# kopacja/rho2sdf.jl

Hardware: AMD Instinct MI355X
Metric: Mvoxels/s SDF extract on 512^3 grid over 100k HEX8; max|err| vs ref (higher is better)
Workload: dtype f64

## Files before the change

### include/rho2sdf_hip.h

```cpp
#ifndef RHO2SDF_HIP_H
#define RHO2SDF_HIP_H

#include <stddef.h>
#include <stdint.h>

#ifdef __cplusplus
extern "C" {
#endif

#define R2S_VERSION 100

#define R2S_OK 0
#define R2S_ERR_ARG (-1)
#define R2S_ERR_NO_DEVICE (-2)
#define R2S_ERR_HIP (-3)
#define R2S_ERR_UNSUPPORTED (-4)
#define R2S_ERR_NOMEM (-5)

#define R2S_HEX8 0
#define R2S_TET4 1

typedef struct {
    double aabb_min[3];
    double aabb_max[3];
// ... 95 lines not shown
void r2s_host_free(void *p);

typedef struct r2s_plan r2s_plan;

int r2s_plan_create(int32_t device, r2s_plan **out);
void r2s_plan_destroy(r2s_plan *plan);

#define R2S_OUT_DIST 1
#define R2S_OUT_SIGN 2
#define R2S_OUT_SDF 4
#define R2S_OUT_XP 8

int r2s_plan_run_dev(r2s_plan *plan, const double *dX, int64_t nnp, const int64_t *dIEN, int64_t nel,
                     const double *d_rho_n, double rho_t, const r2s_grid *grid,
                     const r2s_params *params, int64_t k_begin, int64_t k_end, int32_t mode,
                     double *d_dist, double *d_sign, double *d_sdf, double *d_xp, void *stream,
                     r2s_stats *stats);

int r2s_plan_pack_tiles_dev(r2s_plan *plan, const double *d_local_sdf, double *d_payload, uint32_t *d_ids,
                            int64_t capacity_tiles, int64_t *n_tiles_out, void *stream);
int r2s_unpack_tiles_dev(const double *d_payload, const uint32_t *d_ids, int64_t n_tiles, const r2s_grid *grid,
                         double *d_volume, void *stream);
int r2s_fill_dev(double *d, int64_t n, double value, void *stream);
int r2s_plan_pack_tiles2_dev(r2s_plan *plan, const double *d_local_sdf, double *d_payload, uint32_t *d_ids,
                             int64_t capacity_full, uint64_t *d_masks, uint32_t *d_mask_ids, int64_t capacity_mask,
                             int64_t *n_full_out, int64_t *n_mask_out, void *stream);
int r2s_unpack_masks_dev(const uint64_t *d_masks, const uint32_t *d_mask_ids, int64_t n_tiles, const r2s_grid *grid,
                         double magnitude, double *d_volume, void *stream);

int r2s_unpack_segments_dev(const double *d_buf, int32_t world, int64_t seglen, int64_t cap_full, int64_t cap_mask,
                            const r2s_grid *grid, double magnitude, double *d_volume, void *stream);


int r2s_mesh_volume(const double *X, int64_t nnp, const int64_t *IEN, int64_t nel, int32_t elem_type,
                    const double *rho_e, int32_t device, double *V_domain, double *V_frac);

int r2s_dense_in_nodes(const double *X, int64_t nnp, const int64_t *IEN, int64_t nel, int32_t elem_type,
                       const double *rho_e, int32_t device, double *rho_n_out);

int r2s_find_threshold(const double *X, int64_t nnp, const int64_t *IEN, int64_t nel, const double *rho_n,
                       double target_volume, double tol, int32_t maxit, int32_t device, double *rho_t_out,
                       int32_t *iters_out);

int r2s_find_threshold_et(const double *X, int64_t nnp, const int64_t *IEN, int64_t nel, int32_t elem_type,
                          const double *rho_n, double target_volume, double tol, int32_t maxit, int32_t device,
                          double *rho_t_out, int32_t *iters_out);
// ... 124 lines not shown
```

### rho2sdf.jl_amd/_lib.py

```python
import ctypes
import os

_HERE = os.path.dirname(os.path.abspath(__file__))
LIB_PATH = os.environ.get("R2S_LIB_OVERRIDE") or os.path.join(_HERE, "librho2sdf_hip.so")

c_double_p = ctypes.POINTER(ctypes.c_double)
c_int64_p = ctypes.POINTER(ctypes.c_int64)
c_float_p = ctypes.POINTER(ctypes.c_float)
c_int32_p = ctypes.POINTER(ctypes.c_int32)
OPT_EXTRACT_SURFACE = 0


class R2SGrid(ctypes.Structure):
    _fields_ = [("aabb_min", ctypes.c_double * 3), ("aabb_max", ctypes.c_double * 3),
                ("N", ctypes.c_int64 * 3), ("cell_size", ctypes.c_double), ("ngp", ctypes.c_int64)]


class R2SParams(ctypes.Structure):
    _fields_ = [("band_factor", ctypes.c_double), ("elem_type", ctypes.c_int32),
                ("device", ctypes.c_int32), ("zstride", ctypes.c_int32), ("zphase", ctypes.c_int32),
                ("n_gpus", ctypes.c_int32), ("true_min", ctypes.c_int32), ("sign_no_inner", ctypes.c_int32),
                ("reserved_", ctypes.c_int32)]


# ... 45 lines not shown
_P = ctypes.c_void_p
_MESH = [c_double_p, ctypes.c_int64, c_int64_p, ctypes.c_int64]
_COMMON = _MESH + [c_double_p, ctypes.c_double, ctypes.POINTER(R2SGrid), ctypes.POINTER(R2SParams)]
SYMBOLS = [
    ("r2s_version", ctypes.c_int, []),
    ("r2s_last_error", ctypes.c_char_p, []),
    ("r2s_device_count", ctypes.c_int, []),
    ("r2s_default_params", None, [ctypes.POINTER(R2SParams)]),
    ("r2s_grid_make", ctypes.c_int, [c_double_p, c_double_p, ctypes.c_int64, ctypes.c_int64,
                                     ctypes.POINTER(R2SGrid)]),
    ("r2s_auto_grid", ctypes.c_int, _MESH + [ctypes.c_int32, ctypes.POINTER(R2SGrid), c_double_p]),
    ("r2s_eval_distances", ctypes.c_int, _COMMON + [c_double_p, c_double_p, ctypes.POINTER(R2SStats)]),
    ("r2s_sign_detection", ctypes.c_int, _COMMON + [c_double_p, ctypes.POINTER(R2SStats)]),
    ("r2s_sdf", ctypes.c_int, _COMMON + [c_double_p, ctypes.POINTER(R2SStats)]),
    ("r2s_plan_create", ctypes.c_int, [ctypes.c_int32, ctypes.POINTER(_P)]),
    ("r2s_plan_destroy", None, [_P]),
    ("r2s_plan_run_dev", ctypes.c_int,
     [_P, _P, ctypes.c_int64, _P, ctypes.c_int64, _P, ctypes.c_double, ctypes.POINTER(R2SGrid),
      ctypes.POINTER(R2SParams), ctypes.c_int64, ctypes.c_int64, ctypes.c_int32, _P, _P, _P, _P, _P,
      ctypes.POINTER(R2SStats)]),
    ("r2s_plan_pack_tiles_dev", ctypes.c_int, [_P, _P, _P, _P, ctypes.c_int64, c_int64_p, _P]),
    ("r2s_unpack_tiles_dev", ctypes.c_int, [_P, _P, ctypes.c_int64, ctypes.POINTER(R2SGrid), _P, _P]),
    ("r2s_fill_dev", ctypes.c_int, [_P, ctypes.c_int64, ctypes.c_double, _P]),
    ("r2s_plan_pack_tiles2_dev", ctypes.c_int, [_P, _P, _P, _P, ctypes.c_int64, _P, _P, ctypes.c_int64, c_int64_p,
                                                c_int64_p, _P]),
    ("r2s_unpack_masks_dev", ctypes.c_int, [_P, _P, ctypes.c_int64, ctypes.POINTER(R2SGrid), ctypes.c_double, _P, _P]),
    ("r2s_unpack_segments_dev", ctypes.c_int, [_P, ctypes.c_int32, ctypes.c_int64, ctypes.c_int64, ctypes.c_int64,
                                               ctypes.POINTER(R2SGrid), ctypes.c_double, _P, _P]),
    ("r2s_mesh_volume", ctypes.c_int, _MESH + [ctypes.c_int32, c_double_p, ctypes.c_int32, c_double_p, c_double_p]),
    ("r2s_dense_in_nodes", ctypes.c_int, _MESH + [ctypes.c_int32, c_double_p, ctypes.c_int32, c_double_p]),
    ("r2s_find_threshold", ctypes.c_int, _MESH + [c_double_p, ctypes.c_double, ctypes.c_double, ctypes.c_int32,
                                                  ctypes.c_int32, c_double_p, ctypes.POINTER(ctypes.c_int32)]),
    ("r2s_find_threshold_et", ctypes.c_int, _MESH + [ctypes.c_int32, c_double_p, ctypes.c_double, ctypes.c_double,
                                                     ctypes.c_int32, ctypes.c_int32, c_double_p,
                                                     ctypes.POINTER(ctypes.c_int32)]),
    ("r2s_isocontour_volume", ctypes.c_int, _MESH + [ctypes.c_int32, c_double_p, ctypes.c_double, ctypes.c_int32,
                                                     c_double_p]),
    ("r2s_default_options", None, [ctypes.POINTER(R2SOptions)]),
    ("r2s_rho2sdf", ctypes.c_int, _MESH + [c_double_p, ctypes.POINTER(R2SOptions), ctypes.POINTER(R2SGrid), c_double_p,
                                           c_double_p, c_double_p, c_float_p, ctypes.POINTER(R2SRunInfo)]),
    ("r2s_last_host_phases", None, [c_double_p]),
    ("r2s_host_alloc", ctypes.c_void_p, [ctypes.c_size_t]),
    ("r2s_host_free", None, [ctypes.c_void_p]),
    ("r2s_remove_artifacts", ctypes.c_int, [c_double_p, ctypes.POINTER(R2SGrid), ctypes.c_double, ctypes.c_double,
                                            ctypes.c_int32, c_int64_p]),
    ("r2s_remove_artifacts_dev", ctypes.c_int, [_P, ctypes.POINTER(R2SGrid), ctypes.c_double, ctypes.c_double, _P,
# ... 101 lines not shown
```

### rho2sdf.jl_amd/csrc/rho2sdf_hip.hip

```cpp
#include <hip/hip_runtime.h>

#include <algorithm>
#include <cmath>
#include <cstdarg>
#include <cstddef>
#include <cstdio>
#include <cstring>
#include <initializer_list>
#include <utility>
#include <string>
#include <vector>

#include "../../include/rho2sdf_hip.h"
#include "r2s_common.hpp"
#include "r2s_device_math.hpp"

#include <type_traits>

using namespace r2s;

__constant__ int c_hex_isn[6][4] = {{0, 3, 2, 1}, {0, 1, 5, 4}, {1, 2, 6, 5},
                                    {2, 3, 7, 6}, {3, 0, 4, 7}, {4, 5, 6, 7}};

#define SCAN_BLOCK 256
#define SCAN_ITEMS 16
#define SCAN_TILE (SCAN_BLOCK * SCAN_ITEMS)

struct ScanPair {
    const uint32_t* in[2];
    uint32_t* out[2];
    uint32_t* sums[2];
};
__global__ void __launch_bounds__(SCAN_BLOCK) scan_block_kernel(ScanPair sp, int64_t n)
{
    __shared__ uint32_t wave_sums[SCAN_BLOCK / 64];
    const uint32_t* __restrict__ in = sp.in[blockIdx.y];
    uint32_t* __restrict__ out = sp.out[blockIdx.y];
    uint32_t* __restrict__ block_sums = sp.sums[blockIdx.y];
    const int64_t base = (int64_t)blockIdx.x * SCAN_TILE + (int64_t)threadIdx.x * SCAN_ITEMS;
    uint32_t v[SCAN_ITEMS], sum = 0;
#pragma unroll
    for (int i = 0; i < SCAN_ITEMS; ++i) {
        v[i] = (base + i < n) ? in[base + i] : 0u;
        sum += v[i];
    }
    const int lane = threadIdx.x & 63, wave = threadIdx.x >> 6;
    uint32_t incl = sum;
#pragma unroll
    for (int off = 1; off < 64; off <<= 1) {
        uint32_t t = __shfl_up(incl, off, 64);
        if (lane >= off) incl += t;
    }
    if (lane == 63) wave_sums[wave] = incl;
    __syncthreads();
    uint32_t wave_off = 0, total = 0;
#pragma unroll
    for (int w = 0; w < SCAN_BLOCK / 64; ++w) {
        if (w < wave) wave_off += wave_sums[w];
        total += wave_sums[w];
    }
    uint32_t run = wave_off + incl - sum;
#pragma unroll
    for (int i = 0; i < SCAN_ITEMS; ++i) {
        if (base + i < n) out[base + i] = run;
        run += v[i];
    }
    if (threadIdx.x == 0 && block_sums) block_sums[blockIdx.x] = total;
}

__global__ void scan_add_kernel(ScanPair sp, int64_t n)
{
    uint32_t* __restrict__ out = sp.out[blockIdx.y];
    const int64_t i = (int64_t)blockIdx.x * SCAN_TILE + threadIdx.x;
    const uint32_t add = sp.sums[blockIdx.y][blockIdx.x];
#pragma unroll
    for (int k = 0; k < SCAN_ITEMS; ++k) {
        int64_t j = i + (int64_t)k * SCAN_BLOCK;
        if (j < n) out[j] += add;
    }
}

struct ZeroSet {
    uint32_t* p[4];
    int64_t nwords[4];
};
__global__ void zero_many_kernel(ZeroSet z)
{
    uint32_t* __restrict__ p = z.p[blockIdx.y];
    const int64_t n = z.nwords[blockIdx.y];
    for (int64_t i = (int64_t)blockIdx.x * blockDim.x + threadIdx.x; i < n; i += (int64_t)gridDim.x * blockDim.x) p[i] = 0u;
}
static void zero_many(hipStream_t st, std::initializer_list<std::pair<void*, size_t>> bufs)
{
    ZeroSet z;
    unsigned nb = 0;
    int64_t mx = 0;
    for (const auto& b : bufs) {
        z.p[nb] = static_cast<uint32_t*>(b.first);
        z.nwords[nb] = (int64_t)((b.second + 3) / 4);
        mx = std::max(mx, z.nwords[nb]);
        nb++;
    }
    for (unsigned i = nb; i < 4; ++i) { z.p[i] = nullptr; z.nwords[i] = 0; }
    const unsigned gx = (unsigned)std::min<int64_t>((mx + 1023) / 1024, 2048);
    if (nb && gx) zero_many_kernel<<<dim3(gx, nb), 256, 0, st>>>(z);
}

struct ReadBack {
    const uint32_t* src[8];
    uint32_t n[8];
    uint32_t dst[8];
    int cnt = 0;
    void add(const uint32_t* p, uint32_t words, uint32_t at) { src[cnt] = p; n[cnt] = words; dst[cnt] = at; ++cnt; }
};
struct SpecExpect {
    uint32_t v[16];
    uint32_t on;
};
__global__ void read_back_kernel(ReadBack rb, uint32_t* __restrict__ host, SpecExpect ex, uint32_t* __restrict__ abort_flag)
{
    const int q = threadIdx.x >> 3, w = threadIdx.x & 7;
    if (q < rb.cnt && (uint32_t)w < rb.n[q]) {
        const uint32_t v = rb.src[q][w];
        host[rb.dst[q] + w] = v;
        if (ex.on && v != ex.v[rb.dst[q] + w]) *abort_flag = 1u;
    }
// ... 1355 lines not shown
                    x[2] = grid_coord(g, 2, slab_global_k(sl, kl));
                    inv_map_hex8(E, x, xi);
                    const double m = fmax(fabs(xi[0]), fmax(fabs(xi[1]), fabs(xi[2])));
                    double val = INFINITY;
                    if (m < 1.01) {
                        hex8_shape(xi, N);
                        double rho = 0.0;
#pragma unroll
                        for (int k = 0; k < 8; ++k) rho += N[k] * E.r[k];
                        val = (rho >= rho_t) ? m : -m;
                    }
                    res[tile_slot(st_off, tb, i, j, kl)] = val;
                }
            }
        }
        c = seg_end;
        if (c < c_end) {
            do { ++lo; } while (chunk_off[lo + 1] <= c);
        }
    }
}

#define AT_ITEMS 8
__global__ void __launch_bounds__(256) active_tiles_kernel(const uint32_t* __restrict__ band_cnt,
                                                           const uint32_t* __restrict__ sign_cnt,
                                                           const uint8_t* __restrict__ hot, uint32_t ntiles,
                                                           uint32_t* __restrict__ active_band,
                                                           uint32_t* __restrict__ active_sign,
                                                           uint32_t* __restrict__ active_any,
                                                           uint32_t* __restrict__ active_sonly,
                                                           const uint8_t* __restrict__ tri,
                                                           uint32_t* __restrict__ active_lean,
                                                           uint32_t* __restrict__ active_tri,
                                                           uint32_t* __restrict__ counters)
{
    __shared__ uint32_t s_cnt[6][AT_ITEMS][4], s_base[6], s_max[2];
    if (threadIdx.x < 2) s_max[threadIdx.x] = 0;
    const int lane = threadIdx.x & 63, wave = threadIdx.x >> 6;
    const unsigned long long below = (1ull << lane) - 1ull;
    const uint32_t t0 = blockIdx.x * (256u * AT_ITEMS);
    uint32_t mxb = 0, mxs = 0;
    uint32_t flags[AT_ITEMS];
#pragma unroll
    for (int i = 0; i < AT_ITEMS; ++i) {
        const uint32_t t = t0 + (uint32_t)i * 256u + threadIdx.x;
        const bool in = t < ntiles;
        const uint32_t bc = in ? band_cnt[t] : 0u, sc = in ? sign_cnt[t] : 0u;
        const bool f[3] = {bc != 0, sc != 0 && hot[t] != 0, false};
        const bool ft = f[0] && tri[t] != 0;
        const bool fl[6] = {f[0], f[1], f[0] || f[1], f[1] && !f[0], f[0] && !ft, ft};
        uint32_t fb = 0;
#pragma unroll
        for (int l = 0; l < 6; ++l) {
            const unsigned long long m = __ballot(fl[l]);
            if (lane == 0) s_cnt[l][i][wave] = (uint32_t)__popcll(m);
            fb |= fl[l] ? (1u << l) : 0u;
        }
        flags[i] = fb;
        if (fl[0] && bc > mxb) mxb = bc;
        if (fl[1] && sc > mxs) mxs = sc;
    }
    __syncthreads();
    if (mxb > 64u) atomicMax(&s_max[0], mxb);
    if (mxs > 64u) atomicMax(&s_max[1], mxs);
    if (threadIdx.x < 6) {
        const int idx[6] = {1, 2, 5, 6, 10, 11};
        uint32_t n = 0;
        for (int i = 0; i < AT_ITEMS; ++i)
            for (int w = 0; w < 4; ++w) {
                const uint32_t c = s_cnt[threadIdx.x][i][w];
// ... 377 lines not shown
__global__ void __launch_bounds__(256) unpack_segments_masks_kernel(const double* __restrict__ buf, int64_t seglen, uint32_t cap_full,
                                                                   uint32_t cap_mask, int nx, int ny, int nz, double magnitude,
                                                                   double* __restrict__ volume)
{
    const double* __restrict__ seg = buf + (int64_t)blockIdx.y * seglen;
    const int64_t nf = reinterpret_cast<const int64_t*>(seg)[0], nm = reinterpret_cast<const int64_t*>(seg)[1];
    const uint32_t w = __builtin_amdgcn_readfirstlane((blockIdx.x * blockDim.x + threadIdx.x) >> 6);
    if (nf < 0 || nf > (int64_t)cap_full || nm < 0 || nm > (int64_t)cap_mask || (int64_t)w >= nm) return;
    const uint64_t* __restrict__ masks = reinterpret_cast<const uint64_t*>(seg + 2 + (int64_t)cap_full * 64 + (cap_full + 1) / 2);
    const uint32_t* __restrict__ ids = reinterpret_cast<const uint32_t*>(masks + cap_mask);
    const int lane = threadIdx.x & 63;
    const int ntx = (nx + 3) / 4, nty = (ny + 3) / 4;
    const uint32_t t = ids[w];
    const int tx = t % ntx, ty = (t / ntx) % nty, tz = t / (ntx * nty);
    const int i = tx * 4 + (lane & 3), j = ty * 4 + ((lane >> 2) & 3), k = tz * 4 + (lane >> 4);
    if (i < nx && j < ny && k < nz) volume[((int64_t)k * ny + j) * nx + i] = ((masks[w] >> lane) & 1ull) ? magnitude : -magnitude;
}

struct r2s_plan {
    int device = 0;
    int n_cu = 256;
    DevBuf deg, ine_ptr, ine, cursor, erec, cls, fmask, nitems, item_off, items;
    DevBuf band_cnt, band_off, band_raw, band_ent, sign_cnt, sign_off, sign_raw, sign_ent;
    DevBuf active, active_sign, active_any, active_sonly, active_lean, active_tri, tri, hot, counters, scan_tmp[3], scan_tmp2[3], nchunks, chunk_off, iso_res, iso_res_xp, strag;
    DevBuf perm, wchunks, hardflag;
    DevBuf sbox, s_nchunks, s_chunk_off, sres;
    DevBuf nstore, store_off, s_nstore, s_store_off;
    SlabInfo last_s;
    GridDev last_g;
    uint32_t last_n_any = 0, last_n_band = 0, last_n_sonly = 0;
    bool has_last = false;
    uint32_t* h_pinned = nullptr;
    uint32_t* d_pinned = nullptr;
    struct Spec {
        bool valid = false;
        int64_t key[12] = {0};
        uint32_t v[16] = {0};
    } spec;
    hipEvent_t ev[8] = {nullptr, nullptr, nullptr, nullptr, nullptr, nullptr, nullptr, nullptr};
    hipStream_t st2 = nullptr;
    hipStream_t st3 = nullptr;
    hipEvent_t ev2[8] = {nullptr, nullptr, nullptr, nullptr, nullptr, nullptr, nullptr, nullptr};
    hipEvent_t ev_fast[2] = {nullptr, nullptr};
    bool fast_timed = false;
};

static int scan_exclusive2(r2s_plan* P, const uint32_t* in0, uint32_t* out0, const uint32_t* in1, uint32_t* out1,
                           int64_t n, hipStream_t st, int level = 0, int bank = 0)
{
    DevBuf* tmp = bank ? P->scan_tmp2 : P->scan_tmp;
    if (n <= 0) return 0;
    const unsigned ny = in1 ? 2u : 1u;
    const int64_t nb = (n + SCAN_TILE - 1) / SCAN_TILE;
    ScanPair sp;
    sp.in[0] = in0; sp.out[0] = out0; sp.in[1] = in1; sp.out[1] = out1;
    sp.sums[0] = sp.sums[1] = nullptr;
    if (nb == 1) {
        scan_block_kernel<<<dim3(1, ny), SCAN_BLOCK, 0, st>>>(sp, n);
        return 0;
    }
    if (level >= 3) return fail(R2S_ERR_ARG, "scan too large");
    if (tmp[level].ensure(sizeof(uint32_t) * 2 * (size_t)nb)) return fail(R2S_ERR_NOMEM, "scan workspace");
    sp.sums[0] = tmp[level].as<uint32_t>();
    sp.sums[1] = sp.sums[0] + nb;
    scan_block_kernel<<<dim3((unsigned)nb, ny), SCAN_BLOCK, 0, st>>>(sp, n);
    int rc = scan_exclusive2(P, sp.sums[0], sp.sums[0], in1 ? sp.sums[1] : nullptr, in1 ? sp.sums[1] : nullptr, nb, st,
                             level + 1, bank);
    if (rc) return rc;
    scan_add_kernel<<<dim3((unsigned)nb, ny), SCAN_BLOCK, 0, st>>>(sp, n);
    return 0;
}
static int scan_exclusive(r2s_plan* P, const uint32_t* in, uint32_t* out, int64_t n, hipStream_t st)
{
    return scan_exclusive2(P, in, out, nullptr, nullptr, n, st);
}

extern "C" {

int r2s_version(void) { return R2S_VERSION; }
const char* r2s_last_error(void) { return g_err.c_str(); }

int r2s_device_count(void)
{
    int n = 0;
    if (hipGetDeviceCount(&n) != hipSuccess) {
        (void)hipGetLastError();
        return 0;
    }
    return n;
}

void r2s_default_params(r2s_params* p)
// ... 86 lines not shown
    for (int i = 0; i < 8; ++i) HIP_TRY(hipEventCreate(&P->ev[i]));
    for (int i = 0; i < 8; ++i) HIP_TRY(hipEventCreate(&P->ev2[i]));
    for (int i = 0; i < 2; ++i) HIP_TRY(hipEventCreate(&P->ev_fast[i]));
    {
        int prio_lo = 0, prio_hi = 0;
        HIP_TRY(hipDeviceGetStreamPriorityRange(&prio_lo, &prio_hi));
        (void)prio_lo;
        HIP_TRY(hipStreamCreateWithPriority(&P->st2, hipStreamNonBlocking, prio_hi));
        HIP_TRY(hipStreamCreateWithFlags(&P->st3, hipStreamNonBlocking));
    }
    *out = P;
    return 0;
}

void r2s_plan_destroy(r2s_plan* P)
{
    if (!P) return;
    (void)hipSetDevice(P->device);
    DevBuf* all[] = {&P->deg, &P->ine_ptr, &P->ine, &P->cursor, &P->erec, &P->cls, &P->fmask, &P->nitems,
                     &P->item_off, &P->items, &P->band_cnt, &P->band_off, &P->band_raw, &P->band_ent,
                     &P->sign_cnt, &P->sign_off, &P->sign_raw, &P->sign_ent, &P->active, &P->active_sign, &P->active_any, &P->active_sonly, &P->active_lean, &P->active_tri, &P->tri,
                     &P->hot, &P->counters, &P->nchunks, &P->chunk_off, &P->iso_res, &P->iso_res_xp, &P->strag,
                     &P->perm, &P->wchunks, &P->hardflag, &P->sbox, &P->s_nchunks, &P->s_chunk_off, &P->sres, &P->nstore, &P->store_off, &P->s_nstore, &P->s_store_off,
                     &P->scan_tmp[0], &P->scan_tmp[1], &P->scan_tmp[2], &P->scan_tmp2[0], &P->scan_tmp2[1], &P->scan_tmp2[2]};
    for (DevBuf* b : all) b->release();
    if (P->h_pinned) (void)hipHostFree(P->h_pinned);
    for (int i = 0; i < 8; ++i)
        if (P->ev[i]) (void)hipEventDestroy(P->ev[i]);
    for (int i = 0; i < 8; ++i)
        if (P->ev2[i]) (void)hipEventDestroy(P->ev2[i]);
    for (int i = 0; i < 2; ++i)
        if (P->ev_fast[i]) (void)hipEventDestroy(P->ev_fast[i]);
    if (P->st2) (void)hipStreamDestroy(P->st2);
    if (P->st3) (void)hipStreamDestroy(P->st3);
    delete P;
}


}

static uint32_t iso_straggler_cap(uint32_t n_store)
{
    static const int cap_env = getenv("R2S_ISO_STRAGGLER_CAP") ? atoi(getenv("R2S_ISO_STRAGGLER_CAP")) : 0;
    if (cap_env > 0) return (uint32_t)cap_env;
    const uint64_t slots = 64ull * std::max<uint32_t>(n_store, 1u);
    return (uint32_t)std::max<uint64_t>(slots / 16, std::min<uint64_t>(slots, 1ull << 20));
}
// ... 107 lines not shown
    ENSURE(P->active_sonly, sizeof(uint32_t) * (size_t)ntiles);
    ENSURE(P->active_lean, sizeof(uint32_t) * (size_t)ntiles);
    ENSURE(P->active_tri, sizeof(uint32_t) * (size_t)ntiles);
    ENSURE(P->tri, (size_t)ntiles + 1);
    ENSURE(P->hot, (size_t)ntiles + 1);
    ENSURE(P->counters, 128);
    uint32_t* counters = P->counters.as<uint32_t>();
    const uint32_t* abort_flag = counters + 15;
    const int64_t key[12] = {nnp, nel, (int64_t)ET::NEN, grid->N[0], grid->N[1], grid->N[2], k_begin, k_end,
                             (int64_t)s.G * 65536 + s.r, (int64_t)mode, (int64_t)ntiles, 0};
    static const bool spec_env = !(getenv("R2S_NO_SPECULATION") && atoi(getenv("R2S_NO_SPECULATION")));
    const bool spec = allow_spec && spec_env && P->spec.valid && memcmp(key, P->spec.key, sizeof key) == 0;
    uint32_t cnt[16] = {0};
    SpecExpect ex;
    memset(&ex, 0, sizeof ex);
    for (int q = 0; q < 32; ++q) P->h_pinned[q] = 0u;
    if (spec) {
        memcpy(cnt, P->spec.v, sizeof cnt);
        memcpy(ex.v, P->spec.v, sizeof cnt);
        ex.on = 1u;
    }

    HIP_TRY(hipStreamWaitEvent(st, P->ev2[5], 0));
    HIP_TRY(hipEventRecord(P->ev[0], st));
    zero_many(st, {{P->deg.p, sizeof(uint32_t) * (size_t)(nnp + 1)}, {P->cursor.p, sizeof(uint32_t) * (size_t)(nnp + 1)},
                   {counters, 128}, {P->nitems.p, sizeof(uint32_t) * (size_t)(nel + 1)}});
    HIP_TRY(hipEventRecord(P->ev2[0], st));
    elem_prep_kernel<ET><<<(unsigned)((nel + 127) / 128), 128, 0, st>>>(
        dX, dIEN, d_rho_n, nel, nnp, rho_t, g, P->erec.as<typename ET::Rec>(),
        P->cls.as<uint8_t>(), P->fmask.as<uint32_t>(), P->nitems.as<uint32_t>(), s, delta);
    HIP_TRY(hipEventRecord(P->ev2[5], st));
    HIP_TRY(hipStreamWaitEvent(P->st2, P->ev2[0], 0));
    {
        const int64_t n = nel * ET::NEN;
        node_degree_kernel<<<(unsigned)((n + 255) / 256), 256, 0, P->st2>>>(dIEN, nel, ET::NEN, nnp, P->deg.as<uint32_t>(), (int*)counters);
        int rc = scan_exclusive(P, P->deg.as<uint32_t>(), P->ine_ptr.as<uint32_t>(), nnp + 1, P->st2);
        if (rc) return rc;
        ine_fill_kernel<<<(unsigned)((n + 255) / 256), 256, 0, P->st2>>>(dIEN, nel, ET::NEN, nnp, P->ine_ptr.as<uint32_t>(), P->cursor.as<uint32_t>(), P->ine.as<uint32_t>());
    }
    HIP_TRY(hipEventRecord(P->ev2[1], P->st2));
    if constexpr (std::is_same<typename ET::Rec, ElemRec>::value) {
        HIP_TRY(hipStreamWaitEvent(P->st2, P->ev2[5], 0));
        HIP_TRY(hipStreamWaitEvent(P->st3, P->ev2[5], 0));
        static const int no_inner_env = getenv("R2S_SIGN_NO_INNER") ? atoi(getenv("R2S_SIGN_NO_INNER")) : 0;
        hex_planes_kernel<<<(unsigned)((nel * 6 + 255) / 256), 256, 0, P->st3>>>(P->erec.as<ElemRec>(), nel,
                                                                                 (no_inner_env || prm.sign_no_inner) ? 1 : 0);
        HIP_TRY(hipEventRecord(P->ev2[5], P->st3));
    }
    constexpr bool HEX = std::is_same<typename ET::Rec, ElemRec>::value;
    const double rmax_needed = HEX ? -INFINITY : rho_t - 1e-12 * (fabs(rho_t) + 1.0);
    const bool sign_items = HEX && want_sign && nel > 0;
    ReadBack rb2;
    if constexpr (HEX) {
        if (sign_items) {
            zero_many(P->st2, {{P->sign_cnt.p, sizeof(uint32_t) * (size_t)(ntiles + 1)}, {P->hot.p, (size_t)ntiles + 1}});
            sign_hot_kernel<ElemRec><<<(unsigned)((nel * BIN_LANES + 255) / 256), 256, 0, P->st2>>>(P->erec.as<ElemRec>(), (uint32_t)nel, g, s, rho_t, P->hot.as<uint8_t>());
            sign_bin_kernel<ElemRec, false><<<(unsigned)((nel * BIN_LANES + 255) / 256), 256, 0, P->st2>>>(P->erec.as<ElemRec>(), (uint32_t)nel, g, s, P->sign_cnt.as<uint32_t>(), nullptr, nullptr, P->hot.as<uint8_t>(), abort_flag, rmax_needed);
            int rc = scan_exclusive2(P, P->sign_cnt.as<uint32_t>(), P->sign_off.as<uint32_t>(), nullptr, nullptr, (int64_t)ntiles + 1, P->st2, 0, 1);
            if (rc) return rc;
            ENSURE(P->sbox, sizeof(SignBox) * (size_t)nel);
            ENSURE(P->s_nchunks, sizeof(uint32_t) * (size_t)(nel + 1));
            ENSURE(P->s_chunk_off, sizeof(uint32_t) * (size_t)(nel + 1));
            ENSURE(P->s_nstore, sizeof(uint32_t) * (size_t)(nel + 1));
            ENSURE(P->s_store_off, sizeof(uint32_t) * (size_t)(nel + 1));
            zero_many(P->st2, {{P->s_nchunks.p, sizeof(uint32_t) * (size_t)(nel + 1)}, {P->s_nstore.p, sizeof(uint32_t) * (size_t)(nel + 1)}});
            sign_box_kernel<<<(unsigned)((nel * BIN_LANES + 255) / 256), 256, 0, P->st2>>>(P->erec.as<ElemRec>(), (uint32_t)nel, g, s, P->hot.as<uint8_t>(), P->sbox.as<SignBox>(), P->s_nchunks.as<uint32_t>(), P->s_nstore.as<uint32_t>());
            rc = scan_exclusive2(P, P->s_nchunks.as<uint32_t>(), P->s_chunk_off.as<uint32_t>(), P->s_nstore.as<uint32_t>(),
                                 P->s_store_off.as<uint32_t>(), nel + 1, P->st2, 0, 1);
            if (rc) return rc;
            rb2.add(P->s_chunk_off.as<uint32_t>() + nel, 1, 11);
            rb2.add(P->s_store_off.as<uint32_t>() + nel, 1, 13);
            HIP_TRY(hipEventRecord(P->ev2[7], P->st2));
        }
    }
    HIP_TRY(hipStreamWaitEvent(st, P->ev2[1], 0));
    face_mask_kernel<ET><<<(unsigned)((nel * ET::NES + 255) / 256), 256, 0, st>>>(
        dIEN, nel, P->ine_ptr.as<uint32_t>(), P->ine.as<uint32_t>(), P->cls.as<uint8_t>(), P->fmask.as<uint32_t>(),
        P->nitems.as<uint32_t>(), (const int*)counters);
    {
        int rc = scan_exclusive(P, P->nitems.as<uint32_t>(), P->item_off.as<uint32_t>(), nel + 1, st);
        if (rc) return rc;
    }
    {
        ReadBack rb;
        rb.add(P->item_off.as<uint32_t>() + nel, 1, 0);
        rb.add(counters, 1, 1);
        read_back_kernel<<<1, 64, 0, st>>>(rb, P->d_pinned, ex, counters + 15);
    }
    if (!spec) {
        HIP_TRY(hipStreamSynchronize(st));
        if (P->h_pinned[1]) return fail(R2S_ERR_ARG, "IEN contains node ids outside 1..nnp");
        cnt[0] = P->h_pinned[0];
        cnt[1] = 0;
    }
    const uint32_t n_items = want_dist ? cnt[0] : 0;
    ENSURE(P->items, sizeof(BandItem) * (size_t)std::max<uint32_t>(n_items, 1));
    ENSURE(P->nchunks, sizeof(uint32_t) * (size_t)(n_items + 1));
    ENSURE(P->chunk_off, sizeof(uint32_t) * (size_t)(n_items + 1));
    ENSURE(P->nstore, sizeof(uint32_t) * (size_t)(n_items + 1));
    ENSURE(P->store_off, sizeof(uint32_t) * (size_t)(n_items + 1));
    if (n_items) {
        ENSURE(P->hardflag, (size_t)n_items + 1);
        zero_many(st, {{P->nchunks.p, sizeof(uint32_t) * (size_t)(n_items + 1)}, {P->nstore.p, sizeof(uint32_t) * (size_t)(n_items + 1)},
                       {P->hardflag.p, (size_t)n_items + 1}});
        item_build_kernel<ET><<<(unsigned)((nel + 63) / 64), 64, 0, st>>>(
            P->erec.as<typename ET::Rec>(), P->cls.as<uint8_t>(), P->fmask.as<uint32_t>(), P->item_off.as<uint32_t>(), nel,
            g, s, delta, P->items.as<BandItem>(), P->nchunks.as<uint32_t>(), P->nstore.as<uint32_t>(), P->hardflag.as<uint8_t>(), rho_t, abort_flag);
        const uint32_t* work_counts = P->nchunks.as<uint32_t>();
        if constexpr (std::is_same<typename ET::Rec, ElemRec>::value) {
            ENSURE(P->perm, sizeof(uint32_t) * (size_t)n_items);
            ENSURE(P->wchunks, sizeof(uint32_t) * (size_t)(n_items + 1));
            work_order_kernel<<<1, 1024, 0, st>>>(P->hardflag.as<uint8_t>(), P->nchunks.as<uint32_t>(), n_items,
                                                  P->perm.as<uint32_t>(), P->wchunks.as<uint32_t>());
            work_counts = P->wchunks.as<uint32_t>();
        }
        int rc = scan_exclusive2(P, work_counts, P->chunk_off.as<uint32_t>(), P->nstore.as<uint32_t>(),
                                 P->store_off.as<uint32_t>(), (int64_t)n_items + 1, st);
        if (rc) return rc;
        item_chunks_kernel<<<(n_items + 255) / 256, 256, 0, st>>>(P->items.as<BandItem>(), P->chunk_off.as<uint32_t>(), P->store_off.as<uint32_t>(), n_items);
        rb2.add(P->chunk_off.as<uint32_t>() + n_items, 1, 10);
        rb2.add(P->store_off.as<uint32_t>() + n_items, 1, 12);
    }
    HIP_TRY(hipEventRecord(P->ev[1], st));

    static const bool overlap_env0 = !(getenv("R2S_NO_OVERLAP") && atoi(getenv("R2S_NO_OVERLAP")));
    static const bool early_env = !(getenv("R2S_NO_EARLY_ISO") && atoi(getenv("R2S_NO_EARLY_ISO")));
    bool early_iso = false;
// ... 62 lines not shown
    active_tiles_kernel<<<(ntiles + 256 * AT_ITEMS - 1) / (256 * AT_ITEMS), 256, 0, bs>>>(P->band_cnt.as<uint32_t>(), P->sign_cnt.as<uint32_t>(), P->hot.as<uint8_t>(), ntiles, P->active.as<uint32_t>(), P->active_sign.as<uint32_t>(), P->active_any.as<uint32_t>(), P->active_sonly.as<uint32_t>(), P->tri.as<uint8_t>(), P->active_lean.as<uint32_t>(), P->active_tri.as<uint32_t>(), counters);
    rb2.add(P->band_off.as<uint32_t>() + ntiles, 1, 2);
    rb2.add(P->sign_off.as<uint32_t>() + ntiles, 1, 3);
    rb2.add(counters + 1, 6, 4);
    rb2.add(counters + 10, 2, 14);
    read_back_kernel<<<1, 64, 0, bs>>>(rb2, P->d_pinned, ex, counters + 15);
    if (!spec) {
        HIP_TRY(hipStreamSynchronize(bs));
        for (int q = 2; q < 16; ++q) cnt[q] = P->h_pinned[q];
    }
    const uint32_t n_band = cnt[2], n_sign = cnt[3], n_active = cnt[4], n_active_sign = cnt[5];
    P->last_s = s; P->last_g = g; P->last_n_any = cnt[8]; P->last_n_band = cnt[4]; P->last_n_sonly = cnt[9]; P->has_last = true;
    const uint32_t n_chunks = n_items ? cnt[10] : 0;
    const uint32_t n_store = n_items ? cnt[12] : 0;
    ENSURE(P->iso_res, sizeof(double) * 64 * (size_t)std::max<uint32_t>(n_store, 1));
    const uint32_t n_schunks = sign_items ? cnt[11] : 0;
    const uint32_t n_sstore = sign_items ? cnt[13] : 0;
    if (sign_items) ENSURE(P->sres, sizeof(double) * 64 * (size_t)std::max<uint32_t>(n_sstore, 1));
    if (mode & R2S_OUT_XP) ENSURE(P->iso_res_xp, sizeof(double) * 192 * (size_t)std::max<uint32_t>(n_store, 1));
    ENSURE(P->band_raw, sizeof(uint32_t) * (size_t)std::max<uint32_t>(n_band, 1));
    ENSURE(P->band_ent, sizeof(uint32_t) * (size_t)std::max<uint32_t>(n_band, 1));
    ENSURE(P->sign_raw, sizeof(uint32_t) * (size_t)std::max<uint32_t>(n_sign, 1));
    ENSURE(P->sign_ent, sizeof(uint32_t) * (size_t)std::max<uint32_t>(n_sign, 1));
    zero_many(bs, {{P->band_cnt.p, sizeof(uint32_t) * (size_t)(ntiles + 1)}, {P->sign_cnt.p, sizeof(uint32_t) * (size_t)(ntiles + 1)}});
    if (n_items)
        band_bin_kernel<true><<<(n_items * BIN_LANES + 127) / 128, 128, 0, bs>>>(P->items.as<BandItem>(), n_items, g, s, P->band_cnt.as<uint32_t>(), P->band_off.as<uint32_t>(), P->band_raw.as<uint32_t>(), nullptr, abort_flag);
    if (want_sign)
        sign_bin_kernel<typename ET::Rec, true><<<(unsigned)((nel * BIN_LANES + 255) / 256), 256, 0, bs>>>(P->erec.as<typename ET::Rec>(), (uint32_t)nel, g, s, P->sign_cnt.as<uint32_t>(), P->sign_off.as<uint32_t>(), HEX ? P->sign_raw.as<uint32_t>() : P->sign_ent.as<uint32_t>(), P->hot.as<uint8_t>(), abort_flag, rmax_needed);
    if (n_active) {
        bin_sort_small_kernel<<<(n_active * SORT_LANES + 255) / 256, 256, 0, bs>>>(P->active.as<uint32_t>(), n_active, P->band_off.as<uint32_t>(), P->band_raw.as<uint32_t>(), P->band_ent.as<uint32_t>(), abort_flag);
        if (cnt[6] > 64u)
            bin_sort_kernel<<<(n_active + 3) / 4, 256, 0, bs>>>(P->active.as<uint32_t>(), n_active, P->band_off.as<uint32_t>(), P->band_raw.as<uint32_t>(), P->band_ent.as<uint32_t>(), abort_flag);
    }
    if (n_active_sign && HEX) {
        bin_sort_small_kernel<<<(n_active_sign * SORT_LANES + 255) / 256, 256, 0, bs>>>(P->active_sign.as<uint32_t>(), n_active_sign, P->sign_off.as<uint32_t>(), P->sign_raw.as<uint32_t>(), P->sign_ent.as<uint32_t>(), abort_flag);
        if (cnt[7] > 64u)
            bin_sort_kernel<<<(n_active_sign + 3) / 4, 256, 0, bs>>>(P->active_sign.as<uint32_t>(), n_active_sign, P->sign_off.as<uint32_t>(), P->sign_raw.as<uint32_t>(), P->sign_ent.as<uint32_t>(), abort_flag);
    }
    HIP_TRY(hipEventRecord(P->ev[2], bs));

    static const bool overlap_env = !(getenv("R2S_NO_OVERLAP") && atoi(getenv("R2S_NO_OVERLAP")));
    const bool overlap = !HEX && overlap_env && mode == R2S_OUT_SDF && want_sign && want_dist;
    const bool fork = HEX && overlap_env && want_sign && want_dist && n_chunks && n_schunks;
    {
        const bool two_streams = overlap || fork;
        hipStream_t fs = two_streams ? P->st2 : st;
        const unsigned fill_grid = 256 * 8;
// ... 268 lines not shown
    return 0;
}

int r2s_unpack_segments_dev(const double* d_buf, int32_t world, int64_t seglen, int64_t cap_full, int64_t cap_mask,
                            const r2s_grid* grid, double magnitude, double* d_volume, void* stream)
{
    if (!d_buf || !grid || !d_volume || world < 1 || world > 65535 || cap_full < 0 || cap_mask < 0 ||
        cap_full >= ((int64_t)1 << 31) || cap_mask >= ((int64_t)1 << 31))
        return fail(R2S_ERR_ARG, "r2s_unpack_segments_dev: bad argument");
    const int64_t need = 2 + cap_full * 64 + (cap_full + 1) / 2 + cap_mask + (cap_mask + 1) / 2;
    if (seglen < need) return fail(R2S_ERR_ARG, "segment length %lld < %lld for capacities (%lld, %lld)", (long long)seglen, (long long)need,
                                   (long long)cap_full, (long long)cap_mask);
    const int nx = (int)grid->N[0] + 1, ny = (int)grid->N[1] + 1, nz = (int)grid->N[2] + 1;
    if (cap_full)
        unpack_segments_tiles_kernel<<<dim3((unsigned)((cap_full + 3) / 4), (unsigned)world), 256, 0, (hipStream_t)stream>>>(
            d_buf, seglen, (uint32_t)cap_full, nx, ny, nz, d_volume);
    if (cap_mask)
        unpack_segments_masks_kernel<<<dim3((unsigned)((cap_mask + 3) / 4), (unsigned)world), 256, 0, (hipStream_t)stream>>>(
            d_buf, seglen, (uint32_t)cap_full, (uint32_t)cap_mask, nx, ny, nz, magnitude, d_volume);
    HIP_TRY(hipGetLastError());
    return 0;
}

int r2s_fill_dev(double* d, int64_t n, double value, void* stream)
{
    if (!d || n < 0) return fail(R2S_ERR_ARG, "r2s_fill_dev: bad argument");
    if (n) fill_kernel<<<256 * 8, 256, 0, (hipStream_t)stream>>>(d, n, value);
    HIP_TRY(hipGetLastError());
    return 0;
}

}
```

Measured before the change: 33630.

## Replace multi-level scan with single-pass decoupled-lookback scan and trim zeroing launches

Replaces the recursive three-kernel exclusive scan (block scan, recursive scan of block sums, add pass) with a single-pass decoupled-lookback kernel that uses dynamic tile IDs and per-tile flag/value state, and has the last block reset that state. It also has active_tiles_kernel clear band/sign counts in place so a later zero_many launch can be dropped, and merges several zeroing launches into earlier batched ones. The goal is fewer kernel launches and global round trips on the critical path, in exchange for spin-waiting between blocks and a persistent state buffer that must stay zeroed between calls. A debug scan entry point is added for testing.

New measurement: 33310. No clear change (-0.9%).

```diff
diff --git a/include/rho2sdf_hip.h b/include/rho2sdf_hip.h
--- a/include/rho2sdf_hip.h
+++ b/include/rho2sdf_hip.h
@@ -141,6 +141,8 @@
 int r2s_unpack_tiles_dev(const double *d_payload, const uint32_t *d_ids, int64_t n_tiles, const r2s_grid *grid,
                          double *d_volume, void *stream);
 int r2s_fill_dev(double *d, int64_t n, double value, void *stream);
+int r2s_debug_scan_u32(const uint32_t *in0, uint32_t *out0, const uint32_t *in1, uint32_t *out1, int64_t n,
+                       int32_t device);
 int r2s_plan_pack_tiles2_dev(r2s_plan *plan, const double *d_local_sdf, double *d_payload, uint32_t *d_ids,
                              int64_t capacity_full, uint64_t *d_masks, uint32_t *d_mask_ids, int64_t capacity_mask,
                              int64_t *n_full_out, int64_t *n_mask_out, void *stream);
diff --git a/rho2sdf.jl_amd/_lib.py b/rho2sdf.jl_amd/_lib.py
--- a/rho2sdf.jl_amd/_lib.py
+++ b/rho2sdf.jl_amd/_lib.py
@@ -91,6 +91,7 @@
     ("r2s_plan_pack_tiles_dev", ctypes.c_int, [_P, _P, _P, _P, ctypes.c_int64, c_int64_p, _P]),
     ("r2s_unpack_tiles_dev", ctypes.c_int, [_P, _P, ctypes.c_int64, ctypes.POINTER(R2SGrid), _P, _P]),
     ("r2s_fill_dev", ctypes.c_int, [_P, ctypes.c_int64, ctypes.c_double, _P]),
+    ("r2s_debug_scan_u32", ctypes.c_int, [_P, _P, _P, _P, ctypes.c_int64, ctypes.c_int32]),
     ("r2s_plan_pack_tiles2_dev", ctypes.c_int, [_P, _P, _P, _P, ctypes.c_int64, _P, _P, ctypes.c_int64, c_int64_p,
                                                 c_int64_p, _P]),
     ("r2s_unpack_masks_dev", ctypes.c_int, [_P, _P, ctypes.c_int64, ctypes.POINTER(R2SGrid), ctypes.c_double, _P, _P]),
diff --git a/rho2sdf.jl_amd/csrc/rho2sdf_hip.hip b/rho2sdf.jl_amd/csrc/rho2sdf_hip.hip
--- a/rho2sdf.jl_amd/csrc/rho2sdf_hip.hip
+++ b/rho2sdf.jl_amd/csrc/rho2sdf_hip.hip
@@ -26,25 +26,38 @@
 #define SCAN_ITEMS 16
 #define SCAN_TILE (SCAN_BLOCK * SCAN_ITEMS)
 
+#define SCAN_STATE_HDR 2
+#define SCAN_FLAG_TOTAL 1ull
+#define SCAN_FLAG_PREFIX 2ull
+
 struct ScanPair {
     const uint32_t* in[2];
     uint32_t* out[2];
-    uint32_t* sums[2];
+    uint64_t* state[2];
 };
-__global__ void __launch_bounds__(SCAN_BLOCK) scan_block_kernel(ScanPair sp, int64_t n)
+__global__ void __launch_bounds__(SCAN_BLOCK) scan_lookback_kernel(ScanPair sp, int64_t n)
 {
     __shared__ uint32_t wave_sums[SCAN_BLOCK / 64];
-    const uint32_t* __restrict__ in = sp.in[blockIdx.y];
-    uint32_t* __restrict__ out = sp.out[blockIdx.y];
-    uint32_t* __restrict__ block_sums = sp.sums[blockIdx.y];
-    const int64_t base = (int64_t)blockIdx.x * SCAN_TILE + (int64_t)threadIdx.x * SCAN_ITEMS;
+    __shared__ uint32_t sh_tile, sh_excl;
+    const uint32_t* in = sp.in[blockIdx.y];
+    uint32_t* out = sp.out[blockIdx.y];
+    uint64_t* state = sp.state[blockIdx.y];
+    const uint32_t nb = gridDim.x;
+    const int lane = threadIdx.x & 63, wave = threadIdx.x >> 6;
+    uint32_t tile = 0;
+    if (nb > 1) {
+        if (threadIdx.x == 0)
+            sh_tile = (uint32_t)__hip_atomic_fetch_add(&state[0], 1ull, __ATOMIC_RELAXED, __HIP_MEMORY_SCOPE_AGENT);
+        __syncthreads();
+        tile = sh_tile;
+    }
+    const int64_t base = (int64_t)tile * SCAN_TILE + (int64_t)threadIdx.x * SCAN_ITEMS;
     uint32_t v[SCAN_ITEMS], sum = 0;
 #pragma unroll
     for (int i = 0; i < SCAN_ITEMS; ++i) {
         v[i] = (base + i < n) ? in[base + i] : 0u;
         sum += v[i];
     }
-    const int lane = threadIdx.x & 63, wave = threadIdx.x >> 6;
     uint32_t incl = sum;
 #pragma unroll
     for (int off = 1; off < 64; off <<= 1) {
@@ -59,30 +72,61 @@
         if (w < wave) wave_off += wave_sums[w];
         total += wave_sums[w];
     }
-    uint32_t run = wave_off + incl - sum;
+    uint32_t excl = 0;
+    if (nb > 1) {
+        if (wave == 0) {
+            uint64_t* const tiles = state + SCAN_STATE_HDR;
+            if (lane == 0)
+                __hip_atomic_store(&tiles[tile], ((tile ? SCAN_FLAG_TOTAL : SCAN_FLAG_PREFIX) << 32) | total, __ATOMIC_RELAXED,
+                                   __HIP_MEMORY_SCOPE_AGENT);
+            if (tile) {
+                for (int64_t first = (int64_t)tile - 1;; first -= 64) {
+                    const int64_t t = first - lane;
+                    uint64_t w, has_prefix, counted;
+                    for (;;) {
+                        w = t >= 0 ? __hip_atomic_load(&tiles[t], __ATOMIC_RELAXED, __HIP_MEMORY_SCOPE_AGENT) : SCAN_FLAG_PREFIX << 32;
+                        has_prefix = __ballot((w >> 32) == SCAN_FLAG_PREFIX);
+                        counted = has_prefix ? (2ull << __builtin_ctzll(has_prefix)) - 1ull : ~0ull;
+                        if ((__ballot((w >> 32) == 0ull) & counted) == 0ull) break;
+                        __builtin_amdgcn_s_sleep(1);
+                    }
+                    uint32_t part = ((counted >> lane) & 1ull) ? (uint32_t)w : 0u;
+#pragma unroll
+                    for (int off = 32; off > 0; off >>= 1) part += __shfl_xor(part, off, 64);
+                    excl += part;
+                    if (has_prefix) break;
+                }
+                if (lane == 0)
+                    __hip_atomic_store(&tiles[tile], (SCAN_FLAG_PREFIX << 32) | (uint32_t)(excl + total), __ATOMIC_RELAXED,
+                                       __HIP_MEMORY_SCOPE_AGENT);
+            }
+            if (lane == 0) sh_excl = excl;
+        }
+        __syncthreads();
+        excl = sh_excl;
+    }
+    uint32_t run = excl + wave_off + incl - sum;
 #pragma unroll
     for (int i = 0; i < SCAN_ITEMS; ++i) {
         if (base + i < n) out[base + i] = run;
         run += v[i];
     }
-    if (threadIdx.x == 0 && block_sums) block_sums[blockIdx.x] = total;
-}
-
-__global__ void scan_add_kernel(ScanPair sp, int64_t n)
-{
-    uint32_t* __restrict__ out = sp.out[blockIdx.y];
-    const int64_t i = (int64_t)blockIdx.x * SCAN_TILE + threadIdx.x;
-    const uint32_t add = sp.sums[blockIdx.y][blockIdx.x];
-#pragma unroll
-    for (int k = 0; k < SCAN_ITEMS; ++k) {
-        int64_t j = i + (int64_t)k * SCAN_BLOCK;
-        if (j < n) out[j] += add;
-    }
-}
-
+    if (nb > 1 && wave == 0) {
+        uint32_t last = 0;
+        if (lane == 0)
+            last = __hip_atomic_fetch_add(&state[1], 1ull, __ATOMIC_ACQ_REL, __HIP_MEMORY_SCOPE_AGENT) == (uint64_t)nb - 1ull;
+        if (__shfl(last, 0, 64)) {
+            __builtin_amdgcn_fence(__ATOMIC_ACQUIRE, "agent");
+            for (uint32_t i = lane; i < nb + SCAN_STATE_HDR; i += 64)
+                __hip_atomic_store(&state[i], 0ull, __ATOMIC_RELAXED, __HIP_MEMORY_SCOPE_AGENT);
+        }
+    }
+}
+
+#define ZERO_MAX 8
 struct ZeroSet {
-    uint32_t* p[4];
-    int64_t nwords[4];
+    uint32_t* p[ZERO_MAX];
+    int64_t nwords[ZERO_MAX];
 };
 __global__ void zero_many_kernel(ZeroSet z)
 {
@@ -96,12 +140,13 @@
     unsigned nb = 0;
     int64_t mx = 0;
     for (const auto& b : bufs) {
+        if (!b.first || !b.second) continue;
         z.p[nb] = static_cast<uint32_t*>(b.first);
         z.nwords[nb] = (int64_t)((b.second + 3) / 4);
         mx = std::max(mx, z.nwords[nb]);
         nb++;
     }
-    for (unsigned i = nb; i < 4; ++i) { z.p[i] = nullptr; z.nwords[i] = 0; }
+    for (unsigned i = nb; i < ZERO_MAX; ++i) { z.p[i] = nullptr; z.nwords[i] = 0; }
     const unsigned gx = (unsigned)std::min<int64_t>((mx + 1023) / 1024, 2048);
     if (nb && gx) zero_many_kernel<<<dim3(gx, nb), 256, 0, st>>>(z);
 }
@@ -1503,8 +1548,8 @@
 }
 
 #define AT_ITEMS 8
-__global__ void __launch_bounds__(256) active_tiles_kernel(const uint32_t* __restrict__ band_cnt,
-                                                           const uint32_t* __restrict__ sign_cnt,
+__global__ void __launch_bounds__(256) active_tiles_kernel(uint32_t* __restrict__ band_cnt,
+                                                           uint32_t* __restrict__ sign_cnt,
                                                            const uint8_t* __restrict__ hot, uint32_t ntiles,
                                                            uint32_t* __restrict__ active_band,
                                                            uint32_t* __restrict__ active_sign,
@@ -1527,6 +1572,8 @@
         const uint32_t t = t0 + (uint32_t)i * 256u + threadIdx.x;
         const bool in = t < ntiles;
         const uint32_t bc = in ? band_cnt[t] : 0u, sc = in ? sign_cnt[t] : 0u;
+        if (bc) band_cnt[t] = 0u;
+        if (sc) sign_cnt[t] = 0u;
         const bool f[3] = {bc != 0, sc != 0 && hot[t] != 0, false};
         const bool ft = f[0] && tri[t] != 0;
         const bool fl[6] = {f[0], f[1], f[0] || f[1], f[1] && !f[0], f[0] && !ft, ft};
@@ -1950,7 +1997,7 @@
     int n_cu = 256;
     DevBuf deg, ine_ptr, ine, cursor, erec, cls, fmask, nitems, item_off, items;
     DevBuf band_cnt, band_off, band_raw, band_ent, sign_cnt, sign_off, sign_raw, sign_ent;
-    DevBuf active, active_sign, active_any, active_sonly, active_lean, active_tri, tri, hot, counters, scan_tmp[3], scan_tmp2[3], nchunks, chunk_off, iso_res, iso_res_xp, strag;
+    DevBuf active, active_sign, active_any, active_sonly, active_lean, active_tri, tri, hot, counters, scan_state[2], nchunks, chunk_off, iso_res, iso_res_xp, strag;
     DevBuf perm, wchunks, hardflag;
     DevBuf sbox, s_nchunks, s_chunk_off, sres;
     DevBuf nstore, store_off, s_nstore, s_store_off;
@@ -1973,29 +2020,33 @@
     bool fast_timed = false;
 };
 
+static int scan_reserve(r2s_plan* P, int bank, int64_t n, hipStream_t st)
+{
+    DevBuf& state = P->scan_state[bank ? 1 : 0];
+    const size_t bytes = sizeof(uint64_t) * 2 * ((size_t)((n + SCAN_TILE - 1) / SCAN_TILE) + SCAN_STATE_HDR);
+    if (state.cap >= bytes) return 0;
+    if (state.ensure(bytes)) return fail(R2S_ERR_NOMEM, "scan workspace");
+    HIP_TRY(hipMemsetAsync(state.p, 0, state.cap, st));
+    return 0;
+}
+
 static int scan_exclusive2(r2s_plan* P, const uint32_t* in0, uint32_t* out0, const uint32_t* in1, uint32_t* out1,
-                           int64_t n, hipStream_t st, int level = 0, int bank = 0)
-{
-    DevBuf* tmp = bank ? P->scan_tmp2 : P->scan_tmp;
+                           int64_t n, hipStream_t st, int bank = 0)
+{
     if (n <= 0) return 0;
     const unsigned ny = in1 ? 2u : 1u;
     const int64_t nb = (n + SCAN_TILE - 1) / SCAN_TILE;
     ScanPair sp;
     sp.in[0] = in0; sp.out[0] = out0; sp.in[1] = in1; sp.out[1] = out1;
-    sp.sums[0] = sp.sums[1] = nullptr;
-    if (nb == 1) {
-        scan_block_kernel<<<dim3(1, ny), SCAN_BLOCK, 0, st>>>(sp, n);
-        return 0;
-    }
-    if (level >= 3) return fail(R2S_ERR_ARG, "scan too large");
-    if (tmp[level].ensure(sizeof(uint32_t) * 2 * (size_t)nb)) return fail(R2S_ERR_NOMEM, "scan workspace");
-    sp.sums[0] = tmp[level].as<uint32_t>();
-    sp.sums[1] = sp.sums[0] + nb;
-    scan_block_kernel<<<dim3((unsigned)nb, ny), SCAN_BLOCK, 0, st>>>(sp, n);
-    int rc = scan_exclusive2(P, sp.sums[0], sp.sums[0], in1 ? sp.sums[1] : nullptr, in1 ? sp.sums[1] : nullptr, nb, st,
-                             level + 1, bank);
-    if (rc) return rc;
-    scan_add_kernel<<<dim3((unsigned)nb, ny), SCAN_BLOCK, 0, st>>>(sp, n);
+    sp.state[0] = sp.state[1] = nullptr;
+    if (nb > 1) {
+        const size_t words = (size_t)nb + SCAN_STATE_HDR;
+        const int rc = scan_reserve(P, bank, n, st);
+        if (rc) return rc;
+        sp.state[0] = P->scan_state[bank ? 1 : 0].as<uint64_t>();
+        sp.state[1] = sp.state[0] + words;
+    }
+    scan_lookback_kernel<<<dim3((unsigned)nb, ny), SCAN_BLOCK, 0, st>>>(sp, n);
     return 0;
 }
 static int scan_exclusive(r2s_plan* P, const uint32_t* in, uint32_t* out, int64_t n, hipStream_t st)
@@ -2128,7 +2179,7 @@
                      &P->sign_cnt, &P->sign_off, &P->sign_raw, &P->sign_ent, &P->active, &P->active_sign, &P->active_any, &P->active_sonly, &P->active_lean, &P->active_tri, &P->tri,
                      &P->hot, &P->counters, &P->nchunks, &P->chunk_off, &P->iso_res, &P->iso_res_xp, &P->strag,
                      &P->perm, &P->wchunks, &P->hardflag, &P->sbox, &P->s_nchunks, &P->s_chunk_off, &P->sres, &P->nstore, &P->store_off, &P->s_nstore, &P->s_store_off,
-                     &P->scan_tmp[0], &P->scan_tmp[1], &P->scan_tmp[2], &P->scan_tmp2[0], &P->scan_tmp2[1], &P->scan_tmp2[2]};
+                     &P->scan_state[0], &P->scan_state[1]};
     for (DevBuf* b : all) b->release();
     if (P->h_pinned) (void)hipHostFree(P->h_pinned);
     for (int i = 0; i < 8; ++i)
@@ -2282,9 +2333,22 @@
     }
 
     HIP_TRY(hipStreamWaitEvent(st, P->ev2[5], 0));
+    for (int bank = 0; bank < 2; ++bank) {
+        const int rc = scan_reserve(P, bank, std::max<int64_t>(std::max(nnp, nel), (int64_t)ntiles) + 1, st);
+        if (rc) return rc;
+    }
     HIP_TRY(hipEventRecord(P->ev[0], st));
+    const uint32_t n_items_early = (spec && want_dist) ? cnt[0] : 0u;
+    if (n_items_early) {
+        ENSURE(P->nchunks, sizeof(uint32_t) * (size_t)(n_items_early + 1));
+        ENSURE(P->nstore, sizeof(uint32_t) * (size_t)(n_items_early + 1));
+        ENSURE(P->hardflag, (size_t)n_items_early + 1);
+    }
     zero_many(st, {{P->deg.p, sizeof(uint32_t) * (size_t)(nnp + 1)}, {P->cursor.p, sizeof(uint32_t) * (size_t)(nnp + 1)},
-                   {counters, 128}, {P->nitems.p, sizeof(uint32_t) * (size_t)(nel + 1)}});
+                   {counters, 128}, {P->nitems.p, sizeof(uint32_t) * (size_t)(nel + 1)},
+                   {n_items_early ? P->nchunks.p : nullptr, sizeof(uint32_t) * (size_t)(n_items_early + 1)},
+                   {n_items_early ? P->nstore.p : nullptr, sizeof(uint32_t) * (size_t)(n_items_early + 1)},
+                   {n_items_early ? P->hardflag.p : nullptr, (size_t)n_items_early + 1}});
     HIP_TRY(hipEventRecord(P->ev2[0], st));
     elem_prep_kernel<ET><<<(unsigned)((nel + 127) / 128), 128, 0, st>>>(
         dX, dIEN, d_rho_n, nel, nnp, rho_t, g, P->erec.as<typename ET::Rec>(),
@@ -2313,20 +2377,20 @@
     ReadBack rb2;
     if constexpr (HEX) {
         if (sign_items) {
-            zero_many(P->st2, {{P->sign_cnt.p, sizeof(uint32_t) * (size_t)(ntiles + 1)}, {P->hot.p, (size_t)ntiles + 1}});
-            sign_hot_kernel<ElemRec><<<(unsigned)((nel * BIN_LANES + 255) / 256), 256, 0, P->st2>>>(P->erec.as<ElemRec>(), (uint32_t)nel, g, s, rho_t, P->hot.as<uint8_t>());
-            sign_bin_kernel<ElemRec, false><<<(unsigned)((nel * BIN_LANES + 255) / 256), 256, 0, P->st2>>>(P->erec.as<ElemRec>(), (uint32_t)nel, g, s, P->sign_cnt.as<uint32_t>(), nullptr, nullptr, P->hot.as<uint8_t>(), abort_flag, rmax_needed);
-            int rc = scan_exclusive2(P, P->sign_cnt.as<uint32_t>(), P->sign_off.as<uint32_t>(), nullptr, nullptr, (int64_t)ntiles + 1, P->st2, 0, 1);
-            if (rc) return rc;
             ENSURE(P->sbox, sizeof(SignBox) * (size_t)nel);
             ENSURE(P->s_nchunks, sizeof(uint32_t) * (size_t)(nel + 1));
             ENSURE(P->s_chunk_off, sizeof(uint32_t) * (size_t)(nel + 1));
             ENSURE(P->s_nstore, sizeof(uint32_t) * (size_t)(nel + 1));
             ENSURE(P->s_store_off, sizeof(uint32_t) * (size_t)(nel + 1));
-            zero_many(P->st2, {{P->s_nchunks.p, sizeof(uint32_t) * (size_t)(nel + 1)}, {P->s_nstore.p, sizeof(uint32_t) * (size_t)(nel + 1)}});
+            zero_many(P->st2, {{P->sign_cnt.p, sizeof(uint32_t) * (size_t)(ntiles + 1)}, {P->hot.p, (size_t)ntiles + 1},
+                               {P->s_nchunks.p, sizeof(uint32_t) * (size_t)(nel + 1)}, {P->s_nstore.p, sizeof(uint32_t) * (size_t)(nel + 1)}});
+            sign_hot_kernel<ElemRec><<<(unsigned)((nel * BIN_LANES + 255) / 256), 256, 0, P->st2>>>(P->erec.as<ElemRec>(), (uint32_t)nel, g, s, rho_t, P->hot.as<uint8_t>());
+            sign_bin_kernel<ElemRec, false><<<(unsigned)((nel * BIN_LANES + 255) / 256), 256, 0, P->st2>>>(P->erec.as<ElemRec>(), (uint32_t)nel, g, s, P->sign_cnt.as<uint32_t>(), nullptr, nullptr, P->hot.as<uint8_t>(), abort_flag, rmax_needed);
+            int rc = scan_exclusive2(P, P->sign_cnt.as<uint32_t>(), P->sign_off.as<uint32_t>(), nullptr, nullptr, (int64_t)ntiles + 1, P->st2, 1);
+            if (rc) return rc;
             sign_box_kernel<<<(unsigned)((nel * BIN_LANES + 255) / 256), 256, 0, P->st2>>>(P->erec.as<ElemRec>(), (uint32_t)nel, g, s, P->hot.as<uint8_t>(), P->sbox.as<SignBox>(), P->s_nchunks.as<uint32_t>(), P->s_nstore.as<uint32_t>());
             rc = scan_exclusive2(P, P->s_nchunks.as<uint32_t>(), P->s_chunk_off.as<uint32_t>(), P->s_nstore.as<uint32_t>(),
-                                 P->s_store_off.as<uint32_t>(), nel + 1, P->st2, 0, 1);
+                                 P->s_store_off.as<uint32_t>(), nel + 1, P->st2, 1);
             if (rc) return rc;
             rb2.add(P->s_chunk_off.as<uint32_t>() + nel, 1, 11);
             rb2.add(P->s_store_off.as<uint32_t>() + nel, 1, 13);
@@ -2361,8 +2425,9 @@
     ENSURE(P->store_off, sizeof(uint32_t) * (size_t)(n_items + 1));
     if (n_items) {
         ENSURE(P->hardflag, (size_t)n_items + 1);
-        zero_many(st, {{P->nchunks.p, sizeof(uint32_t) * (size_t)(n_items + 1)}, {P->nstore.p, sizeof(uint32_t) * (size_t)(n_items + 1)},
-                       {P->hardflag.p, (size_t)n_items + 1}});
+        if (!n_items_early)
+            zero_many(st, {{P->nchunks.p, sizeof(uint32_t) * (size_t)(n_items + 1)}, {P->nstore.p, sizeof(uint32_t) * (size_t)(n_items + 1)},
+                           {P->hardflag.p, (size_t)n_items + 1}});
         item_build_kernel<ET><<<(unsigned)((nel + 63) / 64), 64, 0, st>>>(
             P->erec.as<typename ET::Rec>(), P->cls.as<uint8_t>(), P->fmask.as<uint32_t>(), P->item_off.as<uint32_t>(), nel,
             g, s, delta, P->items.as<BandItem>(), P->nchunks.as<uint32_t>(), P->nstore.as<uint32_t>(), P->hardflag.as<uint8_t>(), rho_t, abort_flag);
@@ -2471,7 +2536,6 @@
     ENSURE(P->band_ent, sizeof(uint32_t) * (size_t)std::max<uint32_t>(n_band, 1));
     ENSURE(P->sign_raw, sizeof(uint32_t) * (size_t)std::max<uint32_t>(n_sign, 1));
     ENSURE(P->sign_ent, sizeof(uint32_t) * (size_t)std::max<uint32_t>(n_sign, 1));
-    zero_many(bs, {{P->band_cnt.p, sizeof(uint32_t) * (size_t)(ntiles + 1)}, {P->sign_cnt.p, sizeof(uint32_t) * (size_t)(ntiles + 1)}});
     if (n_items)
         band_bin_kernel<true><<<(n_items * BIN_LANES + 127) / 128, 128, 0, bs>>>(P->items.as<BandItem>(), n_items, g, s, P->band_cnt.as<uint32_t>(), P->band_off.as<uint32_t>(), P->band_raw.as<uint32_t>(), nullptr, abort_flag);
     if (want_sign)
@@ -2786,6 +2850,42 @@
     return 0;
 }
 
+int r2s_debug_scan_u32(const uint32_t* in0, uint32_t* out0, const uint32_t* in1, uint32_t* out1, int64_t n, int32_t device)
+{
+    if (!in0 || !out0 || (in1 != nullptr) != (out1 != nullptr) || n < 1 || n >= (int64_t)1 << 31)
+        return fail(R2S_ERR_ARG, "r2s_debug_scan_u32: bad argument");
+    if (device < 0) device = 0;
+    int rc = check_device(device);
+    if (rc) return rc;
+    HIP_TRY(hipSetDevice(device));
+    const size_t bytes = sizeof(uint32_t) * (size_t)n;
+    r2s_plan P;
+    DevBuf buf[4];
+    const uint32_t* h_in[2] = {in0, in1};
+    uint32_t* h_out[2] = {out0, out1};
+    uint32_t* d_in[2] = {nullptr, nullptr};
+    uint32_t* d_out[2] = {nullptr, nullptr};
+    const int na = in1 ? 2 : 1;
+    hipError_t e = hipSuccess;
+    for (int a = 0; a < na && e == hipSuccess && !rc; ++a) {
+        const bool in_place = h_out[a] == h_in[a];
+        if (buf[2 * a].ensure(bytes) || (!in_place && buf[2 * a + 1].ensure(bytes))) { rc = fail(R2S_ERR_NOMEM, "scan buffers"); break; }
+        d_in[a] = buf[2 * a].as<uint32_t>();
+        d_out[a] = in_place ? d_in[a] : buf[2 * a + 1].as<uint32_t>();
+        e = hipMemcpy(d_in[a], h_in[a], bytes, hipMemcpyHostToDevice);
+    }
+    if (!rc && e == hipSuccess) rc = scan_exclusive2(&P, d_in[0], d_out[0], d_in[1], d_out[1], n, nullptr);
+    if (!rc && e == hipSuccess) e = hipGetLastError();
+    if (!rc && e == hipSuccess) e = hipStreamSynchronize(nullptr);
+    for (int a = 0; a < na && e == hipSuccess && !rc; ++a) e = hipMemcpy(h_out[a], d_out[a], bytes, hipMemcpyDeviceToHost);
+    for (DevBuf& b : buf) b.release();
+    P.scan_state[0].release();
+    P.scan_state[1].release();
+    if (rc) return rc;
+    if (e != hipSuccess) return fail(R2S_ERR_HIP, "r2s_debug_scan_u32: %s", hipGetErrorString(e));
+    return 0;
+}
+
 int r2s_fill_dev(double* d, int64_t n, double value, void* stream)
 {
     if (!d || n < 0) return fail(R2S_ERR_ARG, "r2s_fill_dev: bad argument");
```
